# libav/libav

Hardware: AMD Instinct MI355X
Metric: macroblocks_per_s (higher is better)
Workload: dtype u8

## Files before the change

### libav_amd/csrc/h264_deblock.hip

```cpp
#include <cstdlib>
#include <vector>
#include "h264_deblock_dev.h"

using namespace mi355;

namespace {

#ifdef MI355_PROF
__device__ unsigned long long g_prof[16];
#define PROF_MARK(i) do { const unsigned long long now_ = __builtin_readcyclecounter(); prof_acc[i] += now_ - prof_t; prof_t = now_; } while (0)
#else
#define PROF_MARK(i) do { } while (0)
#endif

#ifndef MI355_DCH_LOG
#define MI355_DCH_LOG 2
#endif
constexpr int DCH_LOG = MI355_DCH_LOG, DCH = 1 << DCH_LOG;
#ifndef MI355_DPAD
#define MI355_DPAD 8
#endif
constexpr int DY_PITCH = 16 * DCH + MI355_DPAD;
constexpr int DC_PITCH = 8 * DCH + MI355_DPAD;
constexpr int DIO_ROWS = 16 / DCH;
// ... 711 lines not shown
                YR(10) = (uint8_t)y14; YR(11) = (uint8_t)y15; YR(12) = (uint8_t)y16; YR(13) = (uint8_t)y17;
            }
            if (chroma_line(u0, u1, u2, u3, byte_of(bsc1, 0), ab_alpha(cab_t), ab_beta(cab_t), byte_of(cct1, 0))) {
                CAR(7) = (uint8_t)u1; CR(0) = (uint8_t)u2;
            }
            if (chroma_line(u4, u5, u6, u7, byte_of(bsc1, 2), ab_alpha(cab_i), ab_beta(cab_i), byte_of(cci1, 2))) {
                CR(3) = (uint8_t)u5; CR(4) = (uint8_t)u6;
            }
#undef YJ
#undef AJ
#undef YR
#undef AR
#undef CR
#undef CAR
        }
    };
    if constexpr (NW == 1) {
        await_above(0);
        dma_issue(0);
        prefetch(pre, 0);
        hl = pre.h;
#pragma nounroll
        for (int t = 0; t < nsteps; t++) {
            agent_drain_stores();
            if (hand && t >= 8) {
                const int done = t - 7 < W ? t - 7 : W;
                if (lane_id() == 0) agent_store_u32(mi355_global_v(prog_self), (uint32_t)done);
            }
            MI355_WAVE_SYNC();
            if (t > 0) stores(t - 1);
            await_above(t + 1);
            dma_issue(t + 1);
            uint32_t bsw0, bsw1, bsc0, bsc1;
            strengths(t, 0, bsw0, bsw1, bsc0, bsc1);
            prefetch(pre, t + 1);
            MI355_WAVE_SYNC();
            edges_v(t, 0, bsw0, bsc0);
            MI355_WAVE_SYNC();
            if (hand) hand_down(t);
            edges_h(t, 0, bsw1, bsc1);
        }
        agent_drain_stores();
        MI355_WAVE_SYNC();
        stores(nsteps - 1);
    } else {
        if (srv_wave) {
            await_above(0);
            dma_issue(0);
            prefetch(pre, 0);
            hl = pre.h;
            uint32_t b[4];
            strengths(0, 0, b[0], b[1], b[2], b[3]);
            *reinterpret_cast<mi355_u32x4 *>(mail->bs[0][lane_id()]) = mi355_u32x4{ b[0], b[1], b[2], b[3] };
            prefetch(pre_next, 1);
        }
#pragma nounroll
        for (int t = 0; t < nsteps; t++) {
            agent_drain_stores();
            if (edge_wave && hand && t >= 8) {
                const int done = t - 7 < W ? t - 7 : W;
                if (lane_id() == 0) agent_store_u32(mi355_global_v(prog_self), (uint32_t)done);
            }
            MI355_WG_BARRIER_LDS();
            if (edge_wave) {
                const mi355_u32x4 b = *reinterpret_cast<const mi355_u32x4 *>(mail->bs[t & 1][lane_id()]);
                edges_v(t, t & 1, b[0], b[2]);
                MI355_WAVE_SYNC();
                if (hand) hand_down(t);
                edges_h(t, t & 1, b[1], b[3]);
            } else {
                pre = pre_next;
                prefetch(pre_next, t + 2);
                if (t > 0) stores(t - 1);
                await_above(t + 1);
                dma_issue(t + 1);
                uint32_t b[4];
                strengths(t + 1, (t + 1) & 1, b[0], b[1], b[2], b[3]);
                *reinterpret_cast<mi355_u32x4 *>(mail->bs[(t + 1) & 1][lane_id()]) = mi355_u32x4{ b[0], b[1], b[2], b[3] };
            }
            MI355_WG_BARRIER_LDS();
        }
        if (!srv_wave) {
            if (hand) {
                agent_drain_stores();
                if (lane_id() == 0) agent_store_u32(mi355_global_v(prog_self), (uint32_t)W);
            }
            return;
        }
        agent_drain_stores();
        stores(nsteps - 1);
        return;
    }
    if (hand) {
        agent_drain_stores();
        if (lane_id() == 0) agent_store_u32(mi355_global_v(prog_self), (uint32_t)W);
    }
}

#ifdef MI355_DB3_WAVES
__attribute__((amdgpu_waves_per_eu(MI355_DB3_WAVES, MI355_DB3_WAVES)))
#endif
__global__ void __launch_bounds__(64)
k_deblock_tiled(const mi355_h264_frame *__restrict__ frames, int nframes, int nbands, uint32_t *sync)
{
    __shared__ Deblock3Lds s;
    uint32_t tk = 0;
    if (lane_id() == 0) tk = atomicAdd(mi355_global(sync), 1u);
    tk = (uint32_t)lane_value((int)tk, 0);
    const int band = (int)(tk / (uint32_t)nframes), pic = (int)(tk - (uint32_t)band * (uint32_t)nframes);
    if (band >= nbands) return;
    const mi355_h264_frame &fr = frames[pic];
    if (4 * band >= uniform(fr.mb_height) || uniform(fr.surface_layout) != MI355_SURFACE_TILED) return;
    uint32_t *prog = mi355_global(sync) + 16 + (size_t)pic * (size_t)nbands;
    if (mi355_global(fr.mv[1]) != nullptr) deblock3_band<true, 1>(s, nullptr, fr, band, prog, 0);
    else deblock3_band<false, 1>(s, nullptr, fr, band, prog, 0);
}
__global__ void __launch_bounds__(128)
k_deblock_tiled2(const mi355_h264_frame *__restrict__ frames, int nframes, int nbands, uint32_t *sync)
{
    __shared__ Deblock3Lds s;
    __shared__ Deblock3Mail mail;
    __shared__ uint32_t ticket;
    if (threadIdx.x == 0) ticket = atomicAdd(mi355_global(sync), 1u);
    __syncthreads();
    const uint32_t tk = (uint32_t)uniform((int)ticket);
    const int wave = uniform((int)(threadIdx.x >> 6));
    const int band = (int)(tk / (uint32_t)nframes), pic = (int)(tk - (uint32_t)band * (uint32_t)nframes);
    if (band >= nbands) return;
    const mi355_h264_frame &fr = frames[pic];
    if (4 * band >= uniform(fr.mb_height) || uniform(fr.surface_layout) != MI355_SURFACE_TILED) return;
    uint32_t *prog = mi355_global(sync) + 16 + (size_t)pic * (size_t)nbands;
    if (mi355_global(fr.mv[1]) != nullptr) deblock3_band<true, 2>(s, &mail, fr, band, prog, wave);
    else deblock3_band<false, 2>(s, &mail, fr, band, prog, wave);
}

}

#ifdef MI355_PROF
extern "C" void mi355_debug_prof(unsigned long long *out, int reset)
{
    unsigned long long z[16] = {};
    MI355_CHECK(hipDeviceSynchronize());
    MI355_CHECK(hipMemcpyFromSymbol(out, HIP_SYMBOL(g_prof), sizeof(z)));
    if (reset) MI355_CHECK(hipMemcpyToSymbol(HIP_SYMBOL(g_prof), z, sizeof(z)));
}
#endif

namespace {
struct SyncBuf {
    int device;
    hipStream_t stream;
    uint32_t *dev;
    size_t words;
};
}
static std::vector<SyncBuf> &sync_pool() { static thread_local std::vector<SyncBuf> pool; return pool; }
uint32_t *mi355::sync_words(hipStream_t st, size_t words)
{
    std::vector<SyncBuf> &pool = sync_pool();
    const int device = mi355::current_device();
    SyncBuf *b = nullptr;
    for (SyncBuf &e : pool)
        if (e.device == device && e.stream == st) { b = &e; break; }
    if (!b) {
        pool.push_back(SyncBuf{ device, st, nullptr, 0 });
        b = &pool.back();
    }
    if (b->dev && b->words >= words) return b->dev;
    if (b->dev) (void)hipFree(b->dev);
    b->dev = nullptr; b->words = 0;
    size_t n = 4096;
    while (n < words) n *= 2;
    if (hipMalloc(reinterpret_cast<void **>(&b->dev), n * sizeof(uint32_t)) != hipSuccess) { b->dev = nullptr; return nullptr; }
    b->words = n;
    return b->dev;
}
void mi355::sync_words_release(hipStream_t st)
{
    std::vector<SyncBuf> &pool = sync_pool();
    const int device = mi355::current_device();
    for (size_t i = 0; i < pool.size(); i++)
        if (pool[i].device == device && pool[i].stream == st) {
            if (pool[i].dev) (void)hipFree(pool[i].dev);
            pool.erase(pool.begin() + (long)i);
            return;
        }
}

namespace {
int deblock_form_pin()
{
    static const int force = std::getenv("MI355_DEBLOCK_FORM") ? std::atoi(std::getenv("MI355_DEBLOCK_FORM")) : 0;
    return force;
}
int deblock_waves_pin()
{
    static const int pin = std::getenv("MI355_DEBLOCK_WAVES") ? std::atoi(std::getenv("MI355_DEBLOCK_WAVES")) : 0;
    return pin;
}
int device_cus()
{
    static int cus = 0;
    if (!cus) {
        hipDeviceProp_t prop;
        int dev = 0;
        cus = hipGetDevice(&dev) == hipSuccess && hipGetDeviceProperties(&prop, dev) == hipSuccess && prop.multiProcessorCount > 0 ? prop.multiProcessorCount : 256;
    }
    return cus;
}
bool linear_form(int kw) { return kw == 1 || kw == 2 || kw == 3 || kw == 4 || kw == 6; }

mi355_h264_deblock_plan_info deblock_plan(int nframes, int max_mb_width, int max_mb_height, int layouts, int cus)
{
    const int nbands = (max_mb_height + 3) / 4, nsteps = max_mb_width + 6;
    const int force = deblock_form_pin();
    mi355_h264_deblock_plan_info p{ 0, 0, 0, 0 };
    const bool tiled_launch = (layouts & MI355_LAYOUTS_TILED) && force == 0;
    if (tiled_launch) {
        const int pin = deblock_waves_pin();
        const long long simds = 4LL * cus;
        p.tiled_waves = pin == 2 || (pin != 1 && (long long)nframes * nbands < 2LL * simds) ? 2 : 1;
        if (!(layouts & MI355_LAYOUTS_LINEAR)) return p;
    }
    int best = 1;
    double best_cost = 0;
    const int forms[5] = { 1, 2, 3, 4, 6 };
    for (int i = 0; i < 5; i++) {
        const int kw = forms[i];
        const long resident = (long)cus * (DEBLOCK_WAVES_PER_CU / kw);
        const double rounds = (double)((nframes + resident - 1) / resident);
        const double cost = rounds * ((nbands + kw - 1) / kw) * (nsteps + DEBLOCK_LAG * (kw - 1)) * (kw > 1 ? 1.25 : 1.0);
        if (i == 0 || cost < best_cost) { best = kw; best_cost = cost; }
    }
    if (linear_form(force)) best = force;
    p.linear_bands = best;
    p.skip_tiled = tiled_launch ? 1 : 0;
    p.linear_launches = (nbands + best - 1) / best;
    return p;
}

int deblock_launch(const mi355_h264_frame *d_frames, int nframes, int nbands, const mi355_h264_deblock_plan_info &p, hipStream_t st)
{
    if (p.tiled_waves) {
        if ((long long)nframes * nbands > 0x7FFFFFFFLL) return -3;
        const size_t words = 16 + (size_t)nframes * (size_t)nbands;
        uint32_t *sync = mi355::sync_words(st, words);
        if (!sync) return -4;
        MI355_TRY(hipMemsetAsync(sync, 0, words * sizeof(uint32_t), st), -4);
        if (p.tiled_waves == 2) hipLaunchKernelGGL(k_deblock_tiled2, dim3((unsigned)(nframes * nbands)), dim3(128), 0, st, d_frames, nframes, nbands, sync);
        else hipLaunchKernelGGL(k_deblock_tiled, dim3((unsigned)(nframes * nbands)), dim3(64), 0, st, d_frames, nframes, nbands, sync);
    }
    for (int band = 0; p.linear_bands && band < nbands; band += p.linear_bands) {
        const dim3 grid((unsigned)nframes);
        switch (p.linear_bands) {
        case 2: hipLaunchKernelGGL(k_deblock_bands<2>, grid, dim3(128), 0, st, d_frames, band, p.skip_tiled); break;
        case 3: hipLaunchKernelGGL(k_deblock_bands<3>, grid, dim3(192), 0, st, d_frames, band, p.skip_tiled); break;
        case 4: hipLaunchKernelGGL(k_deblock_bands<4>, grid, dim3(256), 0, st, d_frames, band, p.skip_tiled); break;
        case 6: hipLaunchKernelGGL(k_deblock_bands<6>, grid, dim3(384), 0, st, d_frames, band, p.skip_tiled); break;
        default: hipLaunchKernelGGL(k_deblock, grid, dim3(64), 0, st, d_frames, band, p.skip_tiled); break;
        }
    }
    return hipGetLastError() == hipSuccess ? 0 : -2;
}
}

extern "C" int mi355_h264_deblock_dev(const mi355_h264_frame *d_frames, int nframes, int max_mb_width, int max_mb_height, void *stream)
{
    return mi355_h264_deblock_layouts_dev(d_frames, nframes, max_mb_width, max_mb_height, MI355_LAYOUTS_LINEAR | MI355_LAYOUTS_TILED, stream);
}

static int deblock_args(const mi355_h264_frame *d_frames, int nframes, int max_mb_width, int max_mb_height, int layouts)
{
    if (!mi355::bind() || !d_frames || nframes <= 0 || !(layouts & (MI355_LAYOUTS_LINEAR | MI355_LAYOUTS_TILED))) return 0;
    const int nbands = (max_mb_height + 3) / 4;
    return nbands <= 0 || max_mb_width <= 0 ? 0 : nbands;
}

extern "C" int mi355_h264_deblock_layouts_dev(const mi355_h264_frame *d_frames, int nframes, int max_mb_width, int max_mb_height, int layouts, void *stream)
{
    const int nbands = deblock_args(d_frames, nframes, max_mb_width, max_mb_height, layouts);
    if (!nbands) return -1;
    return deblock_launch(d_frames, nframes, nbands, deblock_plan(nframes, max_mb_width, max_mb_height, layouts, device_cus()), (hipStream_t)stream);
}

extern "C" int mi355_h264_deblock_plan(int nframes, int max_mb_width, int max_mb_height, int layouts, int cus, mi355_h264_deblock_plan_info *plan)
{
    if (!plan || nframes <= 0 || max_mb_width <= 0 || max_mb_height <= 0 || cus < 0 || !(layouts & (MI355_LAYOUTS_LINEAR | MI355_LAYOUTS_TILED))) return -1;
    if (cus == 0) {
        if (!mi355::bind()) return -1;
        cus = device_cus();
    }
    *plan = deblock_plan(nframes, max_mb_width, max_mb_height, layouts, cus);
    return 0;
}

extern "C" int mi355_h264_deblock_form_dev(const mi355_h264_frame *d_frames, int nframes, int max_mb_width, int max_mb_height, int layouts, int tiled_waves,
                                           int linear_bands, void *stream)
{
    const int nbands = deblock_args(d_frames, nframes, max_mb_width, max_mb_height, layouts);
    if (!nbands) return -1;
    if (tiled_waves < 0 || tiled_waves > 2 || (linear_bands != 0 && !linear_form(linear_bands))) return -1;
    if ((layouts & MI355_LAYOUTS_LINEAR) && !linear_bands) return -1;
    if ((layouts & MI355_LAYOUTS_TILED) && !tiled_waves && !linear_bands) return -1;
    if (tiled_waves && !(layouts & MI355_LAYOUTS_TILED)) return -1;
    const mi355_h264_deblock_plan_info p{ tiled_waves, linear_bands, tiled_waves ? 1 : 0, linear_bands ? (nbands + linear_bands - 1) / linear_bands : 0 };
    return deblock_launch(d_frames, nframes, nbands, p, (hipStream_t)stream);
}
```

### libav_amd/csrc/h264_frame.hip

```cpp
#include <cstdlib>
#include <vector>
#include "h264_recon_dev.h"
#include "../../include/mi355dsp.h"


namespace {

__attribute__((amdgpu_waves_per_eu(MI355_RECON_WAVES, MI355_RECON_WAVES)))
__global__ void __launch_bounds__(64)
k_recon_inter(const mi355_h264_frame *__restrict__ frames, int max_w, int max_h, unsigned long long inv_w, unsigned long long inv_h, int nblocks, int per_xcd)
{
    __shared__ MbLds s;
    recon_inter_wave<false>(s, frames, max_w, max_h, inv_w, inv_h, nblocks, per_xcd);
}
__attribute__((amdgpu_waves_per_eu(MI355_RECON_WAVES, MI355_RECON_WAVES)))
__global__ void __launch_bounds__(64)
k_recon_inter_sparse(const mi355_h264_frame *__restrict__ frames, int max_w, int max_h, unsigned long long inv_w, unsigned long long inv_h, int nblocks, int per_xcd)
{
    __shared__ MbLds s;
    recon_inter_wave<true>(s, frames, max_w, max_h, inv_w, inv_h, nblocks, per_xcd);
}

constexpr int TP = 32;
constexpr int CP = 16;
constexpr int TO = 4;
struct IntraLds {
    MbCore mb;
    __attribute__((aligned(16))) uint8_t tile[17 * TP];
    __attribute__((aligned(16))) uint8_t ctile[2][9 * CP];
    PredScratch ps;
    int dc_t[16];
};
#define TILE(x, y) s.tile[((y) + 1) * TP + (x) + TO]
#define CTILE(p, x, y) s.ctile[p][((y) + 1) * CP + (x) + TO]

__device__ __forceinline__ uint8_t intra_edge_byte(const uint8_t *p, bool agent)
{
    if (!agent) return *p;
    const uintptr_t a = reinterpret_cast<uintptr_t>(p);
    return (uint8_t)(agent_load_u32(reinterpret_cast<const uint32_t *>(a & ~(uintptr_t)3)) >> (8 * (a & 3)));
}
template <bool AGENT>
__device__ __forceinline__ void intra_store_dword(uint8_t *p, uint32_t v)
{
    if (AGENT) agent_store_u32(reinterpret_cast<uint32_t *>(p), v);
    else *reinterpret_cast<uint32_t *>(p) = v;
}
template <bool TILED, bool AGENT>
__device__ __forceinline__ void intra_store_mb(const uint8_t *y, int ypitch, const uint8_t *cb, const uint8_t *cr, int cpitch, const FrameHot &fr, int mb_x, int mb_y)
{
    if (!AGENT) {
        if (TILED) store_mb_pitched_tiled<true>(y, ypitch, cb, cr, cpitch, fr, mb_x, mb_y);
        else store_mb<true>(y, ypitch, cb, cr, cpitch, fr, mb_x, mb_y);
        return;
    }
    const int lane = lane_id();
    const int row = lane >> 2, seg = lane & 3;
    const int plane = (lane >> 4) & 1, crow = (lane >> 1) & 7, cseg = lane & 1;
    const uint32_t vy = tile_dword<true>(y + row * ypitch + 4 * seg), vc = tile_dword<true>((plane ? cr : cb) + crow * cpitch + 4 * cseg);
    if (TILED) {
        intra_store_dword<true>(fr.recon[0] + tile_y_off(mb_x, mb_y, fr.recon_stride[0]) + 4 * lane, vy);
        if (lane < 32) intra_store_dword<true>(fr.recon[1] + tile_c_off(mb_x, mb_y, fr.recon_stride[1]) + 4 * lane, vc);
    } else {
        intra_store_dword<true>(fr.recon[0] + (uint32_t)(__mul24(mb_y * 16 + row, fr.recon_stride[0]) + mb_x * 16 + 4 * seg), vy);
        if (lane < 32) intra_store_dword<true>((plane ? fr.recon[2] : fr.recon[1]) + (uint32_t)(__mul24(mb_y * 8 + crow, fr.recon_stride[1]) + mb_x * 8 + 4 * cseg), vc);
    }
}

template <bool TILED, bool AGENT = false>
__device__ __forceinline__ void recon_intra_mb(IntraLds &s, const mi355_h264_frame &frd, int mb_xy, bool agent_edges = false)
{
    const int lane = lane_id();
    const FrameHot fr = frame_hot(frd);
    const int mb_x = mb_xy % fr.mb_width, mb_y = mb_xy / fr.mb_width;
    const int ys = fr.recon_stride[0], cs = fr.recon_stride[1];
    uint8_t *const ry = fr.recon[0] + (size_t)mb_y * 16 * ys + mb_x * 16;
    const int pic_w = 16 * fr.mb_width;
    const bool top_y = mb_y > 0 && lane < 25 && mb_x * 16 + lane - 1 >= 0 && mb_x * 16 + lane - 1 < pic_w;
    const bool left_y = mb_x > 0 && lane >= 32 && lane < 48;
    const bool top_c = mb_y > 0 && lane < 9 && (mb_x > 0 || lane > 0);
    const bool left_c = mb_x > 0 && lane >= 16 && lane < 24;
    const uint8_t *const rcb = fr.recon[1] + (size_t)mb_y * 8 * cs + mb_x * 8;
    const uint8_t *const rcr = fr.recon[2] + (size_t)mb_y * 8 * cs + mb_x * 8;
    const ptrdiff_t oy = top_y ? (ptrdiff_t)(lane - 1) - ys : (left_y ? (ptrdiff_t)(lane - 32) * ys - 1 : 0);
    const ptrdiff_t oc = top_c ? (ptrdiff_t)(lane - 1) - cs : (left_c ? (ptrdiff_t)(lane - 16) * cs - 1 : 0);
    MbLoad ld;
    load_mb_issue(ld, fr, mb_xy, true, true);
    uint8_t e_y, e_cb, e_cr;
    if (TILED) {
        const int xt = mb_x * 16 + lane - 1, xtc = mb_x * 8 + lane - 1;
        const uint32_t ty = top_y ? tile_y_off(xt >> 4, mb_y - 1, ys) + 15 * 16 + (xt & 15)
                                  : (left_y ? tile_y_off(mb_x - 1, mb_y, ys) + (lane - 32) * 16 + 15 : tile_y_off(mb_x, mb_y, ys));
        const uint32_t tc = top_c ? tile_c_off(xtc >> 3, mb_y - 1, cs) + 7 * 8 + (xtc & 7)
                                  : (left_c ? tile_c_off(mb_x - 1, mb_y, cs) + (lane - 16) * 8 + 7 : tile_c_off(mb_x, mb_y, cs));
        e_y = intra_edge_byte(fr.recon[0] + ty, AGENT && agent_edges); e_cb = intra_edge_byte(fr.recon[1] + tc, AGENT && agent_edges);
        e_cr = intra_edge_byte(fr.recon[1] + tc + 64, AGENT && agent_edges);
    } else {
        e_y = intra_edge_byte(ry + oy, AGENT && agent_edges); e_cb = intra_edge_byte(rcb + oc, AGENT && agent_edges); e_cr = intra_edge_byte(rcr + oc, AGENT && agent_edges);
    }
    MI355_ISSUE_FENCE();
    load_mb_commit(s.mb, ld, true, fr.mv[0] != nullptr, fr.mv[1] != nullptr);
    const mi355_h264_mb &h = s.mb.hdr;
    const uint32_t t = h.mb_type;

    if (t & MI355_MB_INTRA_PCM) {
        const uint8_t *src = reinterpret_cast<const uint8_t *>(s.mb.coef);
        intra_store_mb<TILED, AGENT>(src, 16, src + 256, src + 320, 8, fr, mb_x, mb_y);
        return;
    }
    if (top_y) TILE(lane - 1, -1) = e_y;
    if (left_y) TILE(-1, lane - 32) = e_y;
    if (top_c) { CTILE(0, lane - 1, -1) = e_cb; CTILE(1, lane - 1, -1) = e_cr; }
    if (left_c) { CTILE(0, -1, lane - 16) = e_cb; CTILE(1, -1, lane - 16) = e_cr; }
    MI355_WAVE_SYNC();

    for (int p = 0; p < 2; p++) {
        if (lane < 9) s.ps.T[lane] = CTILE(p, lane - 1, -1);
        if (lane >= 16 && lane < 25) s.ps.L[lane - 16] = CTILE(p, -1, lane - 17);
        MI355_WAVE_SYNC();
        chroma8_pred_fast(s.ps, h.chroma_pred_mode, &CTILE(p, 0, 0), CP);
    }

    if (t & MI355_MB_INTRA16x16) {
        if (lane < 17) s.ps.T[lane] = TILE(lane - 1, -1);
        if (lane >= 32 && lane < 49) s.ps.L[lane - 32] = TILE(-1, lane - 33);
        MI355_WAVE_SYNC();
        intra16_pred_fast(s.ps, h.intra16x16_pred_mode, &TILE(0, 0), TP);
        if ((h.nnz_mask >> MI355_NNZ_LUMA_DC) & 1) {
            const int b4 = lane & 3;
            const int v = s.mb.coef[luma_dc_slot(lane & 15)];
            const int x1 = quad_xor1(v);
            const int w = (b4 & 1) ? x1 - v : v + x1;
            const int y = quad_xor2(w);
            const int tv = b4 == 2 ? y - w : (b4 == 1 ? w - y : w + y);
            if (lane < 16) s.dc_t[(lane & ~3) | (b4 == 1 ? 2 : (b4 == 2 ? 1 : b4))] = tv;
            MI355_WAVE_SYNC();
            if (lane < 16) {
                const int ci = lane >> 2;
                const int t0 = s.dc_t[ci], t1 = s.dc_t[4 + ci], t2 = s.dc_t[8 + ci], t3 = s.dc_t[12 + ci];
                const int ss = t0 + t2, dd = t0 - t2, ee = t1 - t3, uu = t1 + t3;
                const int r = b4 == 0 ? ss + uu : (b4 == 1 ? dd + ee : (b4 == 2 ? dd - ee : ss - uu));
                s.mb.coef[luma_dc_slot(lane)] = (int16_t)((r * (int)h.dc_qmul[0] + 128) >> 8);
            }
            MI355_WAVE_SYNC();
        }
        residual_tile(s.mb, &TILE(0, 0), TP, &CTILE(0, 0, 0), &CTILE(1, 0, 0), CP, true);
    } else if (t & MI355_MB_8x8DCT) {
        for (int i8 = 0; i8 < 4; i8++) {
            const int x0 = 8 * (i8 & 1), y0 = 8 * (i8 >> 1), i = 4 * i8;
            if (lane < 17) s.ps.T[lane] = TILE(x0 + lane - 1, y0 - 1);
            if (lane >= 32 && lane < 41) s.ps.L[lane - 32] = TILE(x0 - 1, y0 + lane - 33);
            MI355_WAVE_SYNC();
            intra_pred_wave(s.ps, 1, h.u.intra4x4_pred_mode[i], (h.topleft_samples_available << i) & 0x8000,
                            (h.topright_samples_available << i) & 0x4000, &TILE(x0, y0), TP);
            int r[8];
            idct8_lds(s.mb.coef + i8 * 64, lane & 7, lane < 8, r);
            if (lane < 8 && ((h.nnz_mask >> i) & 1)) add_col(&TILE(x0 + lane, y0), TP, r, 8);
            MI355_WAVE_SYNC();
        }
    } else {
        for (int i = 0; i < 16; i++) {
            const int x0 = 4 * blk_x4(i), y0 = 4 * blk_y4(i);
            const int tr_ok = (h.topright_samples_available << i) & 0x8000;
            if (lane < 5) s.ps.T[lane] = TILE(x0 + lane - 1, y0 - 1);
            else if (lane < 9) s.ps.T[lane] = tr_ok ? TILE(x0 + lane - 1, y0 - 1) : TILE(x0 + 3, y0 - 1);
            if (lane >= 32 && lane < 37) s.ps.L[lane - 32] = TILE(x0 - 1, y0 + lane - 33);
            MI355_WAVE_SYNC();
            intra_pred_wave(s.ps, 0, h.u.intra4x4_pred_mode[i], 0, 0, &TILE(x0, y0), TP);
            const int q = lane & 3;
            int c[4], r[4], row;
#pragma unroll
            for (int k2 = 0; k2 < 4; k2++) c[k2] = s.mb.coef[i * 16 + q + 4 * k2];
            idct4_quad(c, q, r, row);
            if (lane < 4 && ((h.nnz_mask >> i) & 1)) add_row4<true>(&TILE(x0, y0 + row), r);
            MI355_WAVE_SYNC();
        }
    }
    if (!(t & MI355_MB_INTRA16x16)) residual_chroma<true>(s.mb, &CTILE(0, 0, 0), &CTILE(1, 0, 0), CP);
    intra_store_mb<TILED, AGENT>(&TILE(0, 0), TP, &CTILE(0, 0, 0), &CTILE(1, 0, 0), CP, fr, mb_x, mb_y);
}
#undef TILE

__global__ void __launch_bounds__(64)
k_recon_intra(const mi355_h264_frame *frames, int level, int width)
{
    __shared__ IntraLds s;
    const int f = blockIdx.x / width, k = blockIdx.x - f * width;
    const mi355_h264_frame &frd = frames[f];
    if (level > frd.max_intra_level) return;
    const int first = mi355_global(frd.intra_level_start)[level - 1], count = mi355_global(frd.intra_level_start)[level] - first;
    if (k >= count) return;
    const int mb_xy = (int)mi355_global(frd.intra_list)[first + k];
    if (uniform(frd.surface_layout) == MI355_SURFACE_TILED) recon_intra_mb<true>(s, frd, mb_xy);
    else recon_intra_mb<false>(s, frd, mb_xy);
}

constexpr int INTRA_SINGLE_LEVELS = 16;
constexpr uint32_t INTRA_NAPS_MAX = 1u << 21;
#ifdef MI355_HIP_EMU_H
static inline uint32_t intra_flag_word(const uint8_t *p) { uint32_t v; std::memcpy(&v, reinterpret_cast<const uint8_t *>(reinterpret_cast<uintptr_t>(p) & ~(uintptr_t)3), 4); return v; }
static inline void intra_flag_set(uint8_t *p) { *p = 1; }
#else
__device__ __forceinline__ uint32_t intra_flag_word(const uint8_t *p) { return agent_load_u32(reinterpret_cast<const uint32_t *>(reinterpret_cast<uintptr_t>(p) & ~(uintptr_t)3)); }
__device__ __forceinline__ void intra_flag_set(uint8_t *p) { __hip_atomic_store(p, (uint8_t)1, __ATOMIC_RELAXED, __HIP_MEMORY_SCOPE_AGENT); }
#endif
__global__ void __launch_bounds__(64)
k_recon_intra_all(const mi355_h264_frame *__restrict__ frames, int nframes, int nmb_max, uint8_t *__restrict__ flags, uint32_t *error_word, uint32_t naps_max)
{
    __shared__ IntraLds s;
    const int k = (int)(blockIdx.x / (unsigned)nframes), f = (int)(blockIdx.x - (unsigned)k * (unsigned)nframes);
    const mi355_h264_frame &frd = frames[f];
    const int nlev = uniform(frd.max_intra_level);
    if (nlev <= 0) return;
    if (k >= uniform(mi355_global(frd.intra_level_start)[nlev])) return;
    const int mb_xy = (int)uniform((int)mi355_global(frd.intra_list)[k]);
    const int W = uniform(frd.mb_width), mb_y = mb_xy / W, mb_x = mb_xy - mb_y * W;
    uint8_t *const pic_flags = mi355_global(flags) + (size_t)f * (size_t)nmb_max;
    const int lane = lane_id();
    const int nx = mb_x + (lane == 3 ? 1 : (lane == 2 ? 0 : -1)), ny = mb_y - (lane == 0 ? 0 : 1);
    const bool inside = lane < 4 && nx >= 0 && nx < W && ny >= 0;
    const int nxy = inside ? ny * W + nx : mb_xy;
    const bool dep = inside && (mi355_global_v(reinterpret_cast<const uint32_t *>(mi355_global(frd.mb) + nxy))[0] & MI355_MB_INTRA) != 0;
    static_assert(offsetof(mi355_h264_mb, mb_type) == 0, "the type word of a record");
    const bool waits = __any(dep);
    if (waits) {
        const uint8_t *fp = pic_flags + nxy;
        const int sh = 8 * (int)(reinterpret_cast<uintptr_t>(fp) & 3);
        uint32_t naps = 0;
        while (__any(dep && ((intra_flag_word(fp) >> sh) & 0xFFu) == 0) && naps < naps_max) { wave_nap(); naps++; }
        if (naps >= naps_max && __any(dep && ((intra_flag_word(fp) >> sh) & 0xFFu) == 0) && lane_id() == 0) atomicOr(error_word, (uint32_t)MI355_ERR_WAIT_EXPIRED);
        MI355_ISSUE_FENCE();
    }
    if (uniform(frd.surface_layout) == MI355_SURFACE_TILED) recon_intra_mb<true, true>(s, frd, mb_xy, waits);
    else recon_intra_mb<false, true>(s, frd, mb_xy, waits);
    agent_drain_stores();
    if (lane == 0 && naps_max) intra_flag_set(pic_flags + mb_xy);
}

}

static int recon_inter_launch(const mi355_h264_frame *d_frames, int nframes, int max_mb_width, int max_mb_height, bool sparse, void *stream, int layouts = MI355_LAYOUTS_LINEAR | MI355_LAYOUTS_TILED)
{
    if (!mi355::bind() || !d_frames || nframes <= 0) return -1;
    const int per_frame = max_mb_width * max_mb_height;
    if (per_frame <= 0 || per_frame >= (1 << 24)) return -3;
    const int frames_per_launch = ((1 << 24) - 1) / per_frame;
    const unsigned long long one = 1ull << 40;
    for (int f0 = 0; f0 < nframes; f0 += frames_per_launch) {
        const int nf = nframes - f0 < frames_per_launch ? nframes - f0 : frames_per_launch;
        const int nblocks = nf * per_frame, per_xcd = (nblocks + 7) / 8;
        const unsigned long long iw = (one + max_mb_width - 1) / max_mb_width, ih = (one + max_mb_height - 1) / max_mb_height;
        if (sparse)
            hipLaunchKernelGGL(k_recon_inter_sparse, dim3((unsigned)(8 * per_xcd)), dim3(64), 0, (hipStream_t)stream,
                               d_frames + f0, max_mb_width, max_mb_height, iw, ih, nblocks, per_xcd);
        else if (layouts == MI355_LAYOUTS_TILED) {
            if (!mi355::recon_inter_tiled_launch(d_frames + f0, nf, max_mb_width, max_mb_height, (hipStream_t)stream)) return -4;
        }
        else
            hipLaunchKernelGGL(k_recon_inter, dim3((unsigned)(8 * per_xcd)), dim3(64), 0, (hipStream_t)stream,
                               d_frames + f0, max_mb_width, max_mb_height, iw, ih, nblocks, per_xcd);
    }
    return hipGetLastError() == hipSuccess ? 0 : -2;
}
extern "C" int mi355_h264_recon_inter_dev(const mi355_h264_frame *d_frames, int nframes, int max_mb_width, int max_mb_height, void *stream)
{
    return recon_inter_launch(d_frames, nframes, max_mb_width, max_mb_height, false, stream);
}
extern "C" int mi355_h264_recon_inter_layouts_dev(const mi355_h264_frame *d_frames, int nframes, int max_mb_width, int max_mb_height, int layouts, void *stream)
{
    if (!(layouts & (MI355_LAYOUTS_LINEAR | MI355_LAYOUTS_TILED))) return -1;
    return recon_inter_launch(d_frames, nframes, max_mb_width, max_mb_height, false, stream, layouts);
}
extern "C" int mi355_h264_recon_inter_sparse_dev(const mi355_h264_frame *d_frames, int nframes, int max_mb_width, int max_mb_height, void *stream)
{
    return recon_inter_launch(d_frames, nframes, max_mb_width, max_mb_height, true, stream);
}

extern "C" int mi355_h264_recon_intra_dev(const mi355_h264_frame *d_frames, int nframes, int max_intra_level, int max_level_width, void *stream)
{
    if (!mi355::bind() || !d_frames || nframes <= 0) return -1;
    if (max_intra_level <= 0 || max_level_width <= 0) return 0;
    for (int level = 1; level <= max_intra_level; level++)
        hipLaunchKernelGGL(k_recon_intra, dim3((unsigned)(nframes * max_level_width)), dim3(64), 0, (hipStream_t)stream,
                           d_frames, level, max_level_width);
    return hipGetLastError() == hipSuccess ? 0 : -2;
}

extern "C" int mi355_h264_recon_intra_all_dev(const mi355_h264_frame *d_frames, int nframes, int max_mb_width, int max_mb_height, int max_intra_level, const int32_t *level_widths, void *stream)
{
    if (!mi355::bind() || !d_frames || nframes <= 0 || max_mb_width <= 0 || max_mb_height <= 0 || (max_intra_level > 0 && !level_widths)) return -1;
    static const int single = std::getenv("MI355_INTRA_SINGLE") ? std::atoi(std::getenv("MI355_INTRA_SINGLE")) : -1;
    if (single == 0 || (single != 1 && max_intra_level < INTRA_SINGLE_LEVELS)) return mi355_h264_recon_intra_levels_dev(d_frames, nframes, max_intra_level, level_widths, stream);
    long long per_picture = 0;
    for (int level = 1; level <= max_intra_level; level++) per_picture += level_widths[level - 1] > 0 ? level_widths[level - 1] : 0;
    if (per_picture <= 0) return 0;
    const long long nmb = (long long)max_mb_width * max_mb_height;
    if (per_picture > nmb) per_picture = nmb;
    if ((long long)nframes * per_picture > 0x7FFFFFFFLL || (long long)nframes * nmb > 0x7FFFFFFFLL) return -3;
    const size_t bytes = ((size_t)nframes * (size_t)nmb + 3) & ~(size_t)3;
    uint32_t *flags = mi355::sync_words((hipStream_t)stream, bytes / 4);
    if (!flags) return -4;
    MI355_TRY(hipMemsetAsync(flags, 0, bytes, (hipStream_t)stream), -4);
    uint32_t *err = mi355::error_word();
    if (!err) return -4;
    static const uint32_t naps_max = std::getenv("MI355_INTRA_NAPS_MAX") ? (uint32_t)std::strtoul(std::getenv("MI355_INTRA_NAPS_MAX"), nullptr, 0) : INTRA_NAPS_MAX;
    hipLaunchKernelGGL(k_recon_intra_all, dim3((unsigned)(nframes * per_picture)), dim3(64), 0, (hipStream_t)stream, d_frames, nframes, (int)nmb, reinterpret_cast<uint8_t *>(flags), err, naps_max);
    return hipGetLastError() == hipSuccess ? 0 : -2;
}

extern "C" int mi355_h264_recon_intra_levels_dev(const mi355_h264_frame *d_frames, int nframes, int max_intra_level, const int32_t *level_widths, void *stream)
{
    if (!mi355::bind() || !d_frames || nframes <= 0 || (max_intra_level > 0 && !level_widths)) return -1;
    for (int level = 1; level <= max_intra_level; level++) {
        const int width = level_widths[level - 1];
        if (width <= 0) continue;
        if ((long long)nframes * width > 0x7FFFFFFFLL) return -3;
        hipLaunchKernelGGL(k_recon_intra, dim3((unsigned)(nframes * width)), dim3(64), 0, (hipStream_t)stream, d_frames, level, width);
    }
    return hipGetLastError() == hipSuccess ? 0 : -2;
}

#ifdef MI355_PROF
extern "C" void mi355_debug_rprof(unsigned long long *out, int reset)
{
    unsigned long long z[16] = {};
    MI355_CHECK(hipDeviceSynchronize());
    MI355_CHECK(hipMemcpyFromSymbol(out, HIP_SYMBOL(g_rprof), sizeof(z)));
    if (reset) MI355_CHECK(hipMemcpyToSymbol(HIP_SYMBOL(g_rprof), z, sizeof(z)));
}
#endif

extern "C" int mi355_h264_decode_frames_dev(const mi355_h264_frame *d_frames, int nframes, int max_mb_width, int max_mb_height,
                                            int max_intra_level, int max_level_width, void *stream)
{
    int rc = mi355_h264_recon_inter_dev(d_frames, nframes, max_mb_width, max_mb_height, stream);
    if (rc) return rc;
    rc = mi355_h264_recon_intra_dev(d_frames, nframes, max_intra_level, max_level_width, stream);
    if (rc) return rc;
    return mi355_h264_deblock_dev(d_frames, nframes, max_mb_width, max_mb_height, stream);
}

extern "C" int mi355_h264_decode_frames_layouts_dev(const mi355_h264_frame *d_frames, int nframes, int max_mb_width, int max_mb_height,
                                                    int max_intra_level, const int32_t *level_widths, int layouts, void *stream)
{
    int rc = mi355_h264_recon_inter_layouts_dev(d_frames, nframes, max_mb_width, max_mb_height, layouts, stream);
    if (rc) return rc;
    rc = mi355_h264_recon_intra_all_dev(d_frames, nframes, max_mb_width, max_mb_height, max_intra_level, level_widths, stream);
    if (rc) return rc;
    return mi355_h264_deblock_layouts_dev(d_frames, nframes, max_mb_width, max_mb_height, layouts, stream);
}

extern "C" int mi355_h264_decode_frames_levels_dev(const mi355_h264_frame *d_frames, int nframes, int max_mb_width, int max_mb_height,
                                                   int max_intra_level, const int32_t *level_widths, void *stream)
{
    int rc = mi355_h264_recon_inter_dev(d_frames, nframes, max_mb_width, max_mb_height, stream);
    if (rc) return rc;
    rc = mi355_h264_recon_intra_all_dev(d_frames, nframes, max_mb_width, max_mb_height, max_intra_level, level_widths, stream);
    if (rc) return rc;
    return mi355_h264_deblock_dev(d_frames, nframes, max_mb_width, max_mb_height, stream);
}

namespace {
struct DescStage {
    mi355_h264_frame *host = nullptr, *dev = nullptr;
    size_t cap = 0;
    hipEvent_t copied = nullptr;
    int device = -1;
};
DescStage &desc_stage(int device)
{
    static thread_local std::vector<DescStage> sets;
    for (DescStage &d : sets) if (d.device == device) return d;
    sets.emplace_back();
    sets.back().device = device;
    return sets.back();
}
}
extern "C" int mi355_h264_decode_frames(const mi355_h264_frame *frames, int nframes, void *stream)
{
    if (!mi355::bind() || !frames || nframes <= 0) return -1;
    DescStage &st = desc_stage(mi355::current_device());
    int mw = 0, mh = 0, ml = 0, lw = 0;
    for (int i = 0; i < nframes; i++) {
        if (frames[i].mb_width > mw) mw = frames[i].mb_width;
        if (frames[i].mb_height > mh) mh = frames[i].mb_height;
        if (frames[i].max_intra_level > ml) ml = frames[i].max_intra_level;
        if (frames[i].max_level_width > lw) lw = frames[i].max_level_width;
        if (frames[i].surface_layout != MI355_SURFACE_LINEAR && (frames[i].surface_layout != MI355_SURFACE_TILED || frames[i].field_picture)) return -1;
    }
    if (!st.copied) MI355_TRY(hipEventCreateWithFlags(&st.copied, hipEventDisableTiming), -4);
    else MI355_TRY(hipEventSynchronize(st.copied), -4);
    if ((size_t)nframes > st.cap) {
        size_t ncap = st.cap ? st.cap : 64;
        while (ncap < (size_t)nframes) ncap *= 2;
        if (st.host) (void)hipHostFree(st.host);
        if (st.dev) { MI355_TRY(hipDeviceSynchronize(), -4); (void)hipFree(st.dev); }
        st.host = st.dev = nullptr; st.cap = 0;
        MI355_TRY(hipHostMalloc(reinterpret_cast<void **>(&st.host), sizeof(*st.host) * ncap), -4);
        MI355_TRY(hipMalloc(reinterpret_cast<void **>(&st.dev), sizeof(*st.dev) * ncap), -4);
        st.cap = ncap;
    }
    std::memcpy(st.host, frames, sizeof(*frames) * (size_t)nframes);
    MI355_TRY(hipMemcpyAsync(st.dev, st.host, sizeof(*frames) * (size_t)nframes, hipMemcpyHostToDevice, (hipStream_t)stream), -4);
    MI355_TRY(hipEventRecord(st.copied, (hipStream_t)stream), -4);
    if (ml > 0 && lw <= 0) lw = (mw < mh ? mw : mh) + 1;
    return mi355_h264_decode_frames_dev(st.dev, nframes, mw, mh, ml, lw, stream);
}

static int intra_schedule(mi355_h264_mb *mb, int mb_width, int mb_height, uint32_t *list, int32_t *level_start, int *max_level_width, bool pairs);
extern "C" int mi355_h264_intra_schedule(mi355_h264_mb *mb, int mb_width, int mb_height,
                                         uint32_t *list, int32_t *level_start, int *max_level_width)
{
    return intra_schedule(mb, mb_width, mb_height, list, level_start, max_level_width, false);
}
extern "C" int mi355_h264_intra_schedule_mbaff(mi355_h264_mb *mb, int mb_width, int mb_height,
                                               uint32_t *list, int32_t *level_start, int *max_level_width)
{
    if (mb_height & 1) return -1;
    return intra_schedule(mb, mb_width, mb_height, list, level_start, max_level_width, true);
}
static int intra_schedule(mi355_h264_mb *mb, int mb_width, int mb_height, uint32_t *list, int32_t *level_start, int *max_level_width, bool pairs)
{
    const int nmb = mb_width * mb_height;
    if (!mb || !list || !level_start || nmb <= 0) return -1;
    std::vector<int32_t> level((size_t)nmb, 0), count;
    int maxl = 0;
    for (int i = 0; i < nmb; i++) {
            const int y = pairs ? 2 * (i / (2 * mb_width)) + (i & 1) : i / mb_width, x = pairs ? (i % (2 * mb_width)) >> 1 : i % mb_width;
            const int xy = x + y * mb_width;
            mi355_h264_mb &m = mb[xy];
            if (!(m.mb_type & MI355_MB_INTRA)) { m.intra_level = 0; continue; }
            int lv = 0;
            const int dx[4] = {-1, -1, 0, 1}, dy[4] = {0, -1, -1, -1};
            if (pairs) {
                const int pr = y >> 1;
                for (int k = 0; k < 4; k++)
                    for (int pos = 0; pos < 2; pos++) {
                        const int nx = x + dx[k], ny = 2 * (pr + dy[k]) + pos;
                        if (nx >= 0 && nx < mb_width && ny >= 0 && ny < mb_height && level[(size_t)(nx + ny * mb_width)] > lv)
                            lv = level[(size_t)(nx + ny * mb_width)];
                    }
                if ((y & 1) && level[(size_t)(xy - mb_width)] > lv) lv = level[(size_t)(xy - mb_width)];
            } else
            for (int k = 0; k < 4; k++) {
                const int nx = x + dx[k], ny = y + dy[k];
                if (nx >= 0 && nx < mb_width && ny >= 0 && ny < mb_height && level[(size_t)(nx + ny * mb_width)] > lv)
                    lv = level[(size_t)(nx + ny * mb_width)];
            }
            level[(size_t)xy] = lv + 1;
            m.intra_level = (uint8_t)(lv + 1 > 255 ? 255 : lv + 1);
            if (lv + 1 > maxl) maxl = lv + 1;
        }
    count.assign((size_t)maxl + 2, 0);
    for (int i = 0; i < nmb; i++) if (level[(size_t)i]) count[(size_t)level[(size_t)i]]++;
    int width = 0;
    level_start[0] = 0;
    for (int l = 1; l <= maxl; l++) {
        level_start[l] = level_start[l - 1] + count[(size_t)l];
        if (count[(size_t)l] > width) width = count[(size_t)l];
// ... 154 lines not shown
```

### libav_amd/csrc/mi355_rt.h

```cpp
#ifndef MI355_RT_H
#define MI355_RT_H

#include <hip/hip_runtime.h>
#include <cstdint>
#include <cstddef>
#include <cstdio>
#include <cstdlib>
#include <cstring>

template <class T> __device__ __forceinline__ T *mi355_global(T *p)
{
#if defined(MI355_HIP_EMU_H) || !defined(__HIP_DEVICE_COMPILE__)
    return p;
#else
    const unsigned long long v = (unsigned long long)p;
    const unsigned long long u = (unsigned long long)(unsigned)__builtin_amdgcn_readfirstlane((int)(unsigned)v) |
                                 ((unsigned long long)(unsigned)__builtin_amdgcn_readfirstlane((int)(unsigned)(v >> 32)) << 32);
    auto q = (__attribute__((address_space(1))) T *)u;
    asm("" : "+s"(q));
    return (T *)q;
#endif
}
template <class T> __device__ __forceinline__ T *mi355_global_v(T *p)
{
#if defined(MI355_HIP_EMU_H) || !defined(__HIP_DEVICE_COMPILE__)
    return p;
#else
    auto q = (__attribute__((address_space(1))) T *)p;
    asm("" : "+v"(q));
    return (T *)q;
#endif
}

__device__ __forceinline__ int mi355_inv20(int n)
{
#if defined(MI355_HIP_EMU_H) || !defined(__HIP_DEVICE_COMPILE__)
    return (int)(1048576.0f * (1.0f / (float)n)) + 1;
#else
    return (int)(1048576.0f * __builtin_amdgcn_rcpf((float)n)) + 1;
#endif
}
__device__ __forceinline__ int mi355_div20(int i, int inv) { return (int)(__umul24((unsigned)i, (unsigned)inv) >> 20); }

#if defined(MI355_HIP_EMU_H) || !defined(__HIP_DEVICE_COMPILE__)
#define MI355_ISSUE_FENCE() ((void)0)
#else
#define MI355_ISSUE_FENCE() asm volatile("" ::: "memory")
#endif
#if defined(MI355_HIP_EMU_H) || !defined(__HIP_DEVICE_COMPILE__)
#define MI355_SCHED_BARRIER() ((void)0)
#else
#define MI355_SCHED_BARRIER() __builtin_amdgcn_sched_barrier(0)
#endif
#if defined(MI355_HIP_EMU_H) || !defined(__HIP_DEVICE_COMPILE__)
#define MI355_PIN(v) ((void)(v))
#else
#define MI355_PIN(v) asm volatile("" : "+v"(v))
#endif

#define MI355_CHECK(expr)                                                                    \
    do {                                                                                     \
        hipError_t e_ = (expr);                                                              \
        if (e_ != hipSuccess) {                                                              \
            std::fprintf(stderr, "mi355dsp: %s failed: %s (%s:%d)\n", #expr,                 \
                         hipGetErrorString(e_), __FILE__, __LINE__);                         \
            std::abort();  \
        }                                                                                    \
    } while (0)
#define MI355_TRY(expr, rc)                                                                  \
    do {                                                                                     \
        hipError_t e_ = (expr);                                                              \
        if (e_ != hipSuccess) {                                                              \
            std::fprintf(stderr, "mi355dsp: %s failed: %s (%s:%d)\n", #expr,                 \
                         hipGetErrorString(e_), __FILE__, __LINE__);                         \
            return rc;                                                                       \
        }                                                                                    \
    } while (0)

namespace mi355 {

struct Arena {
    hipStream_t stream = nullptr;
    uint8_t *host = nullptr;
    uint8_t *dev = nullptr;
    size_t cap = 0, used = 0;
    int device = -1;

    void ensure();
    void reset() { used = 0; }
    size_t take(size_t n)
    {
        size_t off = (used + 15) & ~(size_t)15;
        if (off + n > cap) { std::fprintf(stderr, "mi355dsp: staging arena overflow (an entry point did not reserve() its operands)\n"); std::abort(); }
        used = off + n;
        return off;
    }
    void reserve(size_t need) { if (need + 4096 > cap) grow(need + 4096); }
    void grow(size_t need);
    template <typename T> T *h(size_t off) { return reinterpret_cast<T *>(host + off); }
    template <typename T> T *d(size_t off) { return reinterpret_cast<T *>(dev + off); }
    void upload() { MI355_CHECK(hipMemcpyAsync(dev, host, used, hipMemcpyHostToDevice, stream)); }
    void download()
    {
        MI355_CHECK(hipMemcpyAsync(host, dev, used, hipMemcpyDeviceToHost, stream));
        MI355_CHECK(hipStreamSynchronize(stream));
    }
};

Arena &arena();

struct Win {
    size_t off;
    int pitch, wbytes, rows;
};
Win win_pack(Arena &a, const uint8_t *src, ptrdiff_t stride, int wbytes, int rows,
             int valid_w = -1, int valid_rows = -1);
void win_unpack(Arena &a, const Win &w, uint8_t *dst, ptrdiff_t stride, int x0, int y0, int wbytes, int rows);

bool ready();
void sync_words_release(hipStream_t stream);
uint32_t *sync_words(hipStream_t stream, size_t words);
uint32_t *error_word();
int fault_after_wait();
bool blocking_sync();
int current_device();
bool bind();
struct DeviceScope {
    int prev;
    explicit DeviceScope(int device);
    ~DeviceScope();
    DeviceScope(const DeviceScope &) = delete;
    DeviceScope &operator=(const DeviceScope &) = delete;
};

}
#endif
```

Measured before the change: 1.389 billion.

## Use epoch-tagged intra flags and skip waits/publish for first and last levels

Replaces the per-launch memset of the intra dependency flag buffer with a persistent per-stream buffer whose flags are compared against an incrementing epoch, zeroing only every 255 launches or on growth. Adds a BY_LEVEL kernel variant that skips neighbour-wait checks for level-1 macroblocks and skips the agent-scope store path, drain and flag publish for last-level macroblocks. The aim is to drop a memset launch and some synchronisation overhead from the single-kernel intra path. The by-level form is only chosen when its threshold equals the single threshold, so by default it is effectively unreachable unless pinned; the epoch scheme relies on the buffer not being shared with other users.

```diff
diff --git a/libav_amd/csrc/h264_deblock.hip b/libav_amd/csrc/h264_deblock.hip
--- a/libav_amd/csrc/h264_deblock.hip
+++ b/libav_amd/csrc/h264_deblock.hip
@@ -887,20 +887,24 @@
     hipStream_t stream;
     uint32_t *dev;
     size_t words;
+    uint8_t *flags;
+    size_t flag_bytes;
+    uint32_t epoch;
 };
 }
 static std::vector<SyncBuf> &sync_pool() { static thread_local std::vector<SyncBuf> pool; return pool; }
-uint32_t *mi355::sync_words(hipStream_t st, size_t words)
+static SyncBuf *sync_buf(hipStream_t st)
 {
     std::vector<SyncBuf> &pool = sync_pool();
     const int device = mi355::current_device();
-    SyncBuf *b = nullptr;
     for (SyncBuf &e : pool)
-        if (e.device == device && e.stream == st) { b = &e; break; }
-    if (!b) {
-        pool.push_back(SyncBuf{ device, st, nullptr, 0 });
-        b = &pool.back();
-    }
+        if (e.device == device && e.stream == st) return &e;
+    pool.push_back(SyncBuf{ device, st, nullptr, 0, nullptr, 0, 0 });
+    return &pool.back();
+}
+uint32_t *mi355::sync_words(hipStream_t st, size_t words)
+{
+    SyncBuf *b = sync_buf(st);
     if (b->dev && b->words >= words) return b->dev;
     if (b->dev) (void)hipFree(b->dev);
     b->dev = nullptr; b->words = 0;
@@ -910,6 +914,26 @@
     b->words = n;
     return b->dev;
 }
+uint8_t *mi355::intra_flags(hipStream_t st, size_t bytes, uint32_t *epoch)
+{
+    SyncBuf *b = sync_buf(st);
+    bool zero = b->epoch >= 255;
+    if (!b->flags || b->flag_bytes < bytes) {
+        if (b->flags) (void)hipFree(b->flags);
+        b->flags = nullptr; b->flag_bytes = 0;
+        size_t n = 4096;
+        while (n < bytes) n *= 2;
+        if (hipMalloc(reinterpret_cast<void **>(&b->flags), n) != hipSuccess) { b->flags = nullptr; return nullptr; }
+        b->flag_bytes = n;
+        zero = true;
+    }
+    if (zero) {
+        if (hipMemsetAsync(b->flags, 0, b->flag_bytes, st) != hipSuccess) { b->epoch = 255; return nullptr; }
+        b->epoch = 0;
+    }
+    *epoch = ++b->epoch;
+    return b->flags;
+}
 void mi355::sync_words_release(hipStream_t st)
 {
     std::vector<SyncBuf> &pool = sync_pool();
@@ -917,6 +941,7 @@
     for (size_t i = 0; i < pool.size(); i++)
         if (pool[i].device == device && pool[i].stream == st) {
             if (pool[i].dev) (void)hipFree(pool[i].dev);
+            if (pool[i].flags) (void)hipFree(pool[i].flags);
             pool.erase(pool.begin() + (long)i);
             return;
         }
diff --git a/libav_amd/csrc/h264_frame.hip b/libav_amd/csrc/h264_frame.hip
--- a/libav_amd/csrc/h264_frame.hip
+++ b/libav_amd/csrc/h264_frame.hip
@@ -47,9 +47,9 @@
     else *reinterpret_cast<uint32_t *>(p) = v;
 }
 template <bool TILED, bool AGENT>
-__device__ __forceinline__ void intra_store_mb(const uint8_t *y, int ypitch, const uint8_t *cb, const uint8_t *cr, int cpitch, const FrameHot &fr, int mb_x, int mb_y)
-{
-    if (!AGENT) {
+__device__ __forceinline__ void intra_store_mb(const uint8_t *y, int ypitch, const uint8_t *cb, const uint8_t *cr, int cpitch, const FrameHot &fr, int mb_x, int mb_y, bool publish)
+{
+    if (!AGENT || !publish) {
         if (TILED) store_mb_pitched_tiled<true>(y, ypitch, cb, cr, cpitch, fr, mb_x, mb_y);
         else store_mb<true>(y, ypitch, cb, cr, cpitch, fr, mb_x, mb_y);
         return;
@@ -68,7 +68,7 @@
 }
 
 template <bool TILED, bool AGENT = false>
-__device__ __forceinline__ void recon_intra_mb(IntraLds &s, const mi355_h264_frame &frd, int mb_xy, bool agent_edges = false)
+__device__ __forceinline__ void recon_intra_mb(IntraLds &s, const mi355_h264_frame &frd, int mb_xy, bool agent_edges = false, bool publish = true)
 {
     const int lane = lane_id();
     const FrameHot fr = frame_hot(frd);
@@ -105,7 +105,7 @@
 
     if (t & MI355_MB_INTRA_PCM) {
         const uint8_t *src = reinterpret_cast<const uint8_t *>(s.mb.coef);
-        intra_store_mb<TILED, AGENT>(src, 16, src + 256, src + 320, 8, fr, mb_x, mb_y);
+        intra_store_mb<TILED, AGENT>(src, 16, src + 256, src + 320, 8, fr, mb_x, mb_y, publish);
         return;
     }
     if (top_y) TILE(lane - 1, -1) = e_y;
@@ -177,7 +177,7 @@
         }
     }
     if (!(t & MI355_MB_INTRA16x16)) residual_chroma<true>(s.mb, &CTILE(0, 0, 0), &CTILE(1, 0, 0), CP);
-    intra_store_mb<TILED, AGENT>(&TILE(0, 0), TP, &CTILE(0, 0, 0), &CTILE(1, 0, 0), CP, fr, mb_x, mb_y);
+    intra_store_mb<TILED, AGENT>(&TILE(0, 0), TP, &CTILE(0, 0, 0), &CTILE(1, 0, 0), CP, fr, mb_x, mb_y, publish);
 }
 #undef TILE
 
@@ -196,45 +196,54 @@
 }
 
 constexpr int INTRA_SINGLE_LEVELS = 16;
+constexpr int INTRA_BY_LEVEL_FROM = INTRA_SINGLE_LEVELS;
 constexpr uint32_t INTRA_NAPS_MAX = 1u << 21;
 #ifdef MI355_HIP_EMU_H
 static inline uint32_t intra_flag_word(const uint8_t *p) { uint32_t v; std::memcpy(&v, reinterpret_cast<const uint8_t *>(reinterpret_cast<uintptr_t>(p) & ~(uintptr_t)3), 4); return v; }
-static inline void intra_flag_set(uint8_t *p) { *p = 1; }
+static inline void intra_flag_set(uint8_t *p, uint32_t epoch) { *p = (uint8_t)epoch; }
 #else
 __device__ __forceinline__ uint32_t intra_flag_word(const uint8_t *p) { return agent_load_u32(reinterpret_cast<const uint32_t *>(reinterpret_cast<uintptr_t>(p) & ~(uintptr_t)3)); }
-__device__ __forceinline__ void intra_flag_set(uint8_t *p) { __hip_atomic_store(p, (uint8_t)1, __ATOMIC_RELAXED, __HIP_MEMORY_SCOPE_AGENT); }
+__device__ __forceinline__ void intra_flag_set(uint8_t *p, uint32_t epoch) { __hip_atomic_store(p, (uint8_t)epoch, __ATOMIC_RELAXED, __HIP_MEMORY_SCOPE_AGENT); }
 #endif
+template <bool BY_LEVEL>
 __global__ void __launch_bounds__(64)
-k_recon_intra_all(const mi355_h264_frame *__restrict__ frames, int nframes, int nmb_max, uint8_t *__restrict__ flags, uint32_t *error_word, uint32_t naps_max)
+k_recon_intra_all(const mi355_h264_frame *__restrict__ frames, int nframes, int nmb_max, uint8_t *__restrict__ flags, uint32_t *error_word, uint32_t naps_max, uint32_t epoch)
 {
     __shared__ IntraLds s;
     const int k = (int)(blockIdx.x / (unsigned)nframes), f = (int)(blockIdx.x - (unsigned)k * (unsigned)nframes);
     const mi355_h264_frame &frd = frames[f];
     const int nlev = uniform(frd.max_intra_level);
     if (nlev <= 0) return;
-    if (k >= uniform(mi355_global(frd.intra_level_start)[nlev])) return;
+    const int32_t *const level_start = mi355_global(frd.intra_level_start);
+    const int end = uniform(level_start[nlev]), second = BY_LEVEL ? uniform(level_start[1]) : 0, last = BY_LEVEL ? uniform(level_start[nlev - 1]) : end;
+    if (k >= end) return;
+    const bool level1 = k < second, publish = k < last;
     const int mb_xy = (int)uniform((int)mi355_global(frd.intra_list)[k]);
     const int W = uniform(frd.mb_width), mb_y = mb_xy / W, mb_x = mb_xy - mb_y * W;
     uint8_t *const pic_flags = mi355_global(flags) + (size_t)f * (size_t)nmb_max;
     const int lane = lane_id();
-    const int nx = mb_x + (lane == 3 ? 1 : (lane == 2 ? 0 : -1)), ny = mb_y - (lane == 0 ? 0 : 1);
-    const bool inside = lane < 4 && nx >= 0 && nx < W && ny >= 0;
-    const int nxy = inside ? ny * W + nx : mb_xy;
-    const bool dep = inside && (mi355_global_v(reinterpret_cast<const uint32_t *>(mi355_global(frd.mb) + nxy))[0] & MI355_MB_INTRA) != 0;
-    static_assert(offsetof(mi355_h264_mb, mb_type) == 0, "the type word of a record");
-    const bool waits = __any(dep);
-    if (waits) {
-        const uint8_t *fp = pic_flags + nxy;
-        const int sh = 8 * (int)(reinterpret_cast<uintptr_t>(fp) & 3);
-        uint32_t naps = 0;
-        while (__any(dep && ((intra_flag_word(fp) >> sh) & 0xFFu) == 0) && naps < naps_max) { wave_nap(); naps++; }
-        if (naps >= naps_max && __any(dep && ((intra_flag_word(fp) >> sh) & 0xFFu) == 0) && lane_id() == 0) atomicOr(error_word, (uint32_t)MI355_ERR_WAIT_EXPIRED);
-        MI355_ISSUE_FENCE();
-    }
-    if (uniform(frd.surface_layout) == MI355_SURFACE_TILED) recon_intra_mb<true, true>(s, frd, mb_xy, waits);
-    else recon_intra_mb<false, true>(s, frd, mb_xy, waits);
+    bool waits = false;
+    if (!level1) {
+        const int nx = mb_x + (lane == 3 ? 1 : (lane == 2 ? 0 : -1)), ny = mb_y - (lane == 0 ? 0 : 1);
+        const bool inside = lane < 4 && nx >= 0 && nx < W && ny >= 0;
+        const int nxy = inside ? ny * W + nx : mb_xy;
+        const bool dep = inside && (mi355_global_v(reinterpret_cast<const uint32_t *>(mi355_global(frd.mb) + nxy))[0] & MI355_MB_INTRA) != 0;
+        static_assert(offsetof(mi355_h264_mb, mb_type) == 0, "the type word of a record");
+        waits = __any(dep);
+        if (waits) {
+            const uint8_t *fp = pic_flags + nxy;
+            const int sh = 8 * (int)(reinterpret_cast<uintptr_t>(fp) & 3);
+            uint32_t naps = 0;
+            while (__any(dep && ((intra_flag_word(fp) >> sh) & 0xFFu) != epoch) && naps < naps_max) { wave_nap(); naps++; }
+            if (naps >= naps_max && __any(dep && ((intra_flag_word(fp) >> sh) & 0xFFu) != epoch) && lane_id() == 0) atomicOr(error_word, (uint32_t)MI355_ERR_WAIT_EXPIRED);
+            MI355_ISSUE_FENCE();
+        }
+    }
+    if (uniform(frd.surface_layout) == MI355_SURFACE_TILED) recon_intra_mb<true, true>(s, frd, mb_xy, waits, publish);
+    else recon_intra_mb<false, true>(s, frd, mb_xy, waits, publish);
+    if (!publish) return;
     agent_drain_stores();
-    if (lane == 0 && naps_max) intra_flag_set(pic_flags + mb_xy);
+    if (lane == 0 && naps_max) intra_flag_set(pic_flags + mb_xy, epoch);
 }
 
 }
@@ -289,22 +298,26 @@
 extern "C" int mi355_h264_recon_intra_all_dev(const mi355_h264_frame *d_frames, int nframes, int max_mb_width, int max_mb_height, int max_intra_level, const int32_t *level_widths, void *stream)
 {
     if (!mi355::bind() || !d_frames || nframes <= 0 || max_mb_width <= 0 || max_mb_height <= 0 || (max_intra_level > 0 && !level_widths)) return -1;
-    static const int single = std::getenv("MI355_INTRA_SINGLE") ? std::atoi(std::getenv("MI355_INTRA_SINGLE")) : -1;
-    if (single == 0 || (single != 1 && max_intra_level < INTRA_SINGLE_LEVELS)) return mi355_h264_recon_intra_levels_dev(d_frames, nframes, max_intra_level, level_widths, stream);
+    const char *const pin = std::getenv("MI355_INTRA_SINGLE");
+    const int single = pin ? std::atoi(pin) : -1;
+    const bool pinned = single == 0 || single == 1 || single == 2;
+    const int form = pinned ? single : (max_intra_level >= INTRA_SINGLE_LEVELS ? 1 : (max_intra_level >= 2 && max_intra_level >= INTRA_BY_LEVEL_FROM ? 2 : 0));
+    if (form == 0) return mi355_h264_recon_intra_levels_dev(d_frames, nframes, max_intra_level, level_widths, stream);
     long long per_picture = 0;
     for (int level = 1; level <= max_intra_level; level++) per_picture += level_widths[level - 1] > 0 ? level_widths[level - 1] : 0;
     if (per_picture <= 0) return 0;
     const long long nmb = (long long)max_mb_width * max_mb_height;
     if (per_picture > nmb) per_picture = nmb;
     if ((long long)nframes * per_picture > 0x7FFFFFFFLL || (long long)nframes * nmb > 0x7FFFFFFFLL) return -3;
-    const size_t bytes = ((size_t)nframes * (size_t)nmb + 3) & ~(size_t)3;
-    uint32_t *flags = mi355::sync_words((hipStream_t)stream, bytes / 4);
+    uint32_t epoch = 0;
+    uint8_t *flags = mi355::intra_flags((hipStream_t)stream, (size_t)nframes * (size_t)nmb + 3, &epoch);
     if (!flags) return -4;
-    MI355_TRY(hipMemsetAsync(flags, 0, bytes, (hipStream_t)stream), -4);
     uint32_t *err = mi355::error_word();
     if (!err) return -4;
     static const uint32_t naps_max = std::getenv("MI355_INTRA_NAPS_MAX") ? (uint32_t)std::strtoul(std::getenv("MI355_INTRA_NAPS_MAX"), nullptr, 0) : INTRA_NAPS_MAX;
-    hipLaunchKernelGGL(k_recon_intra_all, dim3((unsigned)(nframes * per_picture)), dim3(64), 0, (hipStream_t)stream, d_frames, nframes, (int)nmb, reinterpret_cast<uint8_t *>(flags), err, naps_max);
+    const dim3 grid((unsigned)(nframes * per_picture));
+    if (form == 2) hipLaunchKernelGGL(k_recon_intra_all<true>, grid, dim3(64), 0, (hipStream_t)stream, d_frames, nframes, (int)nmb, flags, err, naps_max, epoch);
+    else hipLaunchKernelGGL(k_recon_intra_all<false>, grid, dim3(64), 0, (hipStream_t)stream, d_frames, nframes, (int)nmb, flags, err, naps_max, epoch);
     return hipGetLastError() == hipSuccess ? 0 : -2;
 }
 
diff --git a/libav_amd/csrc/mi355_rt.h b/libav_amd/csrc/mi355_rt.h
--- a/libav_amd/csrc/mi355_rt.h
+++ b/libav_amd/csrc/mi355_rt.h
@@ -120,6 +120,7 @@
 bool ready();
 void sync_words_release(hipStream_t stream);
 uint32_t *sync_words(hipStream_t stream, size_t words);
+uint8_t *intra_flags(hipStream_t stream, size_t bytes, uint32_t *epoch);
 uint32_t *error_word();
 int fault_after_wait();
 bool blocking_sync();
```

New measurement: 1.388 billion, median of 5. Within noise of the previous version (-0.1%).
